# duongve13112002/DiffusionSpatialControl

Measured on AMD Instinct MI355X. Metric: 512x512 images/sec, SD1.5 25-step DPM++2M Karras with region-biased cross-attention, higher is better.
Workload: dtype f16; 1 GPU; SD1.5 512x512, 25-step DPM++2M Karras, CFG 7.5, 2 region masks, 1 image(s) per generation, 2 generation(s) in flight per GPU; images_per_gpu=1, parallelism=dp1 (independent images, no per-step collective), hip_graph=True, outputs_finite=True, full=False

## Files before the change

### diffusionspatialcontrol_amd/_lib.py

```python
import ctypes
import os
import re

_HERE = os.path.dirname(os.path.abspath(__file__))
_LIB = None


class DscLibraryError(RuntimeError):
    pass


def lib_path():
    return os.environ.get("DSC_LIB_PATH") or os.path.join(_HERE, "libdsc_hip.so")


def header_path():
    return os.path.join(os.path.dirname(_HERE), "include", "dsc_hip.h")


def declared_symbols():
    txt = open(header_path()).read()
    txt = re.sub(r"/\*.*?\*/", "", txt, flags=re.S)
    return sorted(set(re.findall(r"\b(dsc_[a-z0-9_]+)\s*\(", txt)))

# ... 47 lines not shown
                                    [ctypes.c_float, ctypes.c_int, ctypes.c_int, _vp, ctypes.c_size_t, _vp]),
    "dsc_set_workspace_slot": (ctypes.c_int, [ctypes.c_int]),
    "dsc_set_tuning_profile": (ctypes.c_int, [ctypes.c_int]),
    "dsc_get_tuning_profile": (ctypes.c_int, []),
    "dsc_linear_lt_stats": (None, [_vp]),
    "dsc_has_library_gemm": (ctypes.c_int, []),
    "dsc_add_bias_residual": (ctypes.c_int, [_vp] * 4 + [ctypes.c_int64, ctypes.c_int, ctypes.c_int, _vp]),
    "dsc_linear_f16": (ctypes.c_int, [_vp] * 5 + [ctypes.c_int64, ctypes.c_int, ctypes.c_int] + [ctypes.c_int64] * 3 +
                       [ctypes.c_int, ctypes.c_int, _vp]),
    "dsc_debug_set_conv_stamps": (None, [_vp]),
    "dsc_debug_set_conv_ring": (None, [ctypes.c_int]),
    "dsc_conv3x3_supported": (ctypes.c_int, [ctypes.c_int] * 5),
    "dsc_conv3x3_workspace_bytes": (ctypes.c_size_t, [ctypes.c_int] * 6),
    "dsc_conv3x3_nhwc_f16": (ctypes.c_int, [_vp] * 5 + [ctypes.c_int] * 5 + [ctypes.c_int64] * 3 +
                             [ctypes.c_int, ctypes.c_int, ctypes.c_int, ctypes.c_int, _vp, ctypes.c_size_t, _vp]),
    "dsc_conv3x3_fewcin_f16": (ctypes.c_int, [_vp] * 4 + [ctypes.c_int] * 6 + [_vp]),
    "dsc_linear_lt_f16": (ctypes.c_int, [_vp] * 5 + [ctypes.c_int64, ctypes.c_int, ctypes.c_int] + [ctypes.c_int64] * 3 +
                          [ctypes.c_int, _vp]),
    "dsc_linear_rows_f16": (ctypes.c_int, [_vp] * 4 + [ctypes.c_int] * 3 + [ctypes.c_int64] * 2 + [ctypes.c_int, ctypes.c_int, _vp]),
    "dsc_linear_ln_f16": (ctypes.c_int, [_vp] * 5 + [ctypes.c_int64, ctypes.c_int, ctypes.c_int] + [ctypes.c_int64] * 3 +
                          [ctypes.c_int, _vp, ctypes.c_int, _vp, ctypes.c_float, _vp, ctypes.c_int, _vp]),
    "dsc_debug_set_gemm_stages": (None, [ctypes.c_int]),
    "dsc_linear_qkv_f16": (ctypes.c_int, [_vp] * 5 + [ctypes.c_int64, ctypes.c_int, ctypes.c_int, ctypes.c_int64, ctypes.c_int64,
                                          ctypes.c_int, ctypes.c_int, _vp, ctypes.c_int, _vp, ctypes.c_float, ctypes.c_int, _vp]),
    "dsc_add_layernorm": (ctypes.c_int, [_vp] * 6 + [ctypes.c_int64, ctypes.c_int, ctypes.c_float, ctypes.c_int, _vp]),
    "dsc_geglu": (ctypes.c_int, [_vp, _vp, ctypes.c_int64, ctypes.c_int, ctypes.c_int, _vp]),
    "dsc_linear_splitk_workspace_bytes": (ctypes.c_size_t, [ctypes.c_int64, ctypes.c_int, ctypes.c_int, ctypes.c_int]),
    "dsc_linear_splitk_f16": (ctypes.c_int, [_vp] * 5 + [ctypes.c_int64, ctypes.c_int, ctypes.c_int] + [ctypes.c_int64] * 3 +
                              [ctypes.c_int, _vp, ctypes.c_size_t, ctypes.c_int, _vp]),
    "dsc_conv3x3_gn_rows": (ctypes.c_int, [ctypes.c_int] * 7),
# ... 56 lines not shown
```

### diffusionspatialcontrol_amd/csrc/conv3x3.hip

```cpp
#include "dsc_common.h"
#include "dsc_hip.h"
#include "gn_partials.h"
#include <type_traits>

extern int g_dsc_tuning_profile;

namespace {

constexpr int BM = 128, BN = 64, BK = 64, T = 256;
constexpr int kBStageBytes = BN * BK * 2;
constexpr int kAPiecesMax = 25;
constexpr int kABytes = kAPiecesMax * 1024;
constexpr int kRingOff = 0;
constexpr int a_off(int S) { return S * kBStageBytes; }
constexpr int pad_off(int S) { return a_off(S) + 2 * kABytes; }
constexpr int lds_bytes(int S) { return pad_off(S) + 1024; }
constexpr int kEpiStride = BN + 4;
constexpr unsigned kOob = 0x80000000u;

struct ConvParams {
    const half_t* x; const half_t* w; const half_t* bias; const half_t* res; half_t* out; float* ws;
    int B, H, W, Cin, Cout;
    int up;
    int sh, sw;
    int nchw;
    int sub2;
    int oh, ow;
    long long onpix;
    long long ldx, ldr, ldo;
    int nc, splits, cps;
    int order;
// ... 7 lines not shown
    const half_t* add; long long add_ld;
    float* gn_part; int gn_cpg, gn_G;
};

__device__ __forceinline__ void dma16(__amdgpu_buffer_rsrc_t rsrc, unsigned voff, unsigned soff, unsigned lds_byte) {
    __builtin_amdgcn_raw_ptr_buffer_load_lds(rsrc, (__attribute__((address_space(3))) void*)(uintptr_t)lds_byte, 16, voff, soff, 0, 0);
}

template <int N>
__device__ __forceinline__ void wait_vm() {
    static_assert(N >= 0 && N < 64, "vmcnt is 6 bits");
    __builtin_amdgcn_s_waitcnt((N & 15) | (7 << 4) | (15 << 8) | ((N >> 4) << 14));
    asm volatile("" ::: "memory");
}

template <int S>
constexpr int younger_dmas(int t) {
    int n = 0;
    for (int i = 1; i <= S - 2; ++i) n += ((t - i) % 9 + 9) % 9 == 0 ? 9 : 2;
    return n;
}
template <int S>
__device__ __forceinline__ void wait_step(int t) {
    switch (t) {
        case 0: wait_vm<younger_dmas<S>(0)>(); break;
        case 1: wait_vm<younger_dmas<S>(1)>(); break;
        case 2: wait_vm<younger_dmas<S>(2)>(); break;
        case 3: wait_vm<younger_dmas<S>(3)>(); break;
        case 4: wait_vm<younger_dmas<S>(4)>(); break;
        case 5: wait_vm<younger_dmas<S>(5)>(); break;
        case 6: wait_vm<younger_dmas<S>(6)>(); break;
        case 7: wait_vm<younger_dmas<S>(7)>(); break;
        default: wait_vm<younger_dmas<S>(8)>(); break;
    }
}

template <int TW>
__device__ __forceinline__ int halo_swz(int hy, int hx) {
    if constexpr (TW == 16) return (hx >> 1) & 7;
    else return ((hx >> 1) ^ ((hy & 1) << 2)) & 7;
}

struct Frags { h8_t w[4], x0[4], x1[4]; };

__device__ __forceinline__ h8_t lds_read(unsigned byte_addr) {
    return *reinterpret_cast<const __attribute__((address_space(3))) h8_t*>((uintptr_t)byte_addr);
}

template <int TW, int S, int NLOAD = 0>
__global__ __launch_bounds__(T + 64 * NLOAD, (S == 3 || NLOAD ? 2 : 1)) void conv3x3_kernel(ConvParams p) {
    static_assert(S == 3 || S == 9, "the ring depth must divide the 9 taps");
    static_assert(NLOAD == 0 || NLOAD == 4, "loader waves mirror the four computing waves' DMA shares");
    constexpr bool LOADER = NLOAD > 0;
    constexpr int kAOff = a_off(S), kPadOff = pad_off(S);
    constexpr int NSB = 16 / TW;
    constexpr int HWD = TW + 2;
    constexpr int HS = 10 * HWD;
    constexpr int NSLOT = NSB * HS;
    constexpr int NPIECE = (NSLOT + 7) / 8;
    constexpr int NPAR = TW == 16 ? 1 : 2;
    constexpr int MT1 = (32 / TW) * HWD * 128;
    static_assert(NPIECE <= kAPiecesMax && NPIECE <= 28, "halo does not fit");

    extern __shared__ __attribute__((aligned(16))) char smem[];

    const int lane = threadIdx.x & 63, wave_all = __builtin_amdgcn_readfirstlane(threadIdx.x >> 6);
    const bool is_loader = LOADER && wave_all >= 4;
    const int wave = wave_all & 3;
    const int r = lane & 31, hh = lane >> 5;
    const int wm = wave >> 1, wn = wave & 1;

    const int total = p.mt * p.nt * p.splits;
    const int per = gridDim.x >> 3;
    const int v = (blockIdx.x & 7) * per + (blockIdx.x >> 3);
    if (v >= total) return;
    long long st0 = 0, st1 = 0, st2 = 0, sc0 = 0, sc1 = 0, sc2 = 0;
    if (p.stamps) { st0 = __builtin_amdgcn_s_memrealtime(); sc0 = __builtin_amdgcn_s_memtime(); }
    int bm, bn, sp;
    if (p.order) {
        const int rest = fdiv(v, p.fd_nt);
        bn = v - rest * p.nt;
        sp = fdiv(rest, p.fd_mt); bm = rest - sp * p.mt;
    } else {
        const int rest = fdiv(v, p.fd_mt);
        bm = v - rest * p.mt;
        sp = fdiv(rest, p.fd_nt); bn = rest - sp * p.nt;
    }
    const int n0 = bn * BN;
    const int cb = sp * p.cps, ce = min(p.nc, cb + p.cps);
    const int ns = (ce - cb) * 9;

    const __amdgpu_buffer_rsrc_t xr = __builtin_amdgcn_make_buffer_rsrc(const_cast<half_t*>(p.x), 0, p.x_bytes, 0x00020000);
    const __amdgpu_buffer_rsrc_t wr = __builtin_amdgcn_make_buffer_rsrc(const_cast<half_t*>(p.w), 0, p.w_bytes, 0x00020000);

    unsigned wvoff[2];
#pragma unroll
    for (int pc = 0; pc < 2; ++pc) {
        const int row = (pc * 4 + wave) * 8 + (lane >> 3);
        const int chunk = (lane & 7) ^ ((row >> 1) & 7);
        wvoff[pc] = ((unsigned)(n0 + row) * 9u * (unsigned)p.Cin + chunk * 8) * 2u;
    }
    auto issue_b = [&](unsigned soff, int stage) {
#pragma unroll
        for (int pc = 0; pc < 2; ++pc) dma16(wr, wvoff[pc], soff, kRingOff + stage * kBStageBytes + (pc * 4 + wave) * 1024);
    };
    auto tile_soff = [&](int c, int t) { return ((unsigned)t * (unsigned)p.Cin + (unsigned)c * BK) * 2u; };

    const bool dma_wave = !LOADER || is_loader;
    if (dma_wave) {
#pragma unroll
        for (int k = 0; k < S; ++k) issue_b(tile_soff(cb, k), k);
    }

    int ob[NSB], oy[NSB], ox[NSB];
#pragma unroll
// ... 11 lines not shown
        if (slot < NSLOT) {
            const int sb = slot / HS, rem = slot % HS;
            const int hy = rem / HWD, hx = rem % HWD;
            const int b = NSB == 1 ? ob[0] : (sb ? ob[NSB - 1] : ob[0]);
            const int y = (NSB == 1 ? oy[0] : (sb ? oy[NSB - 1] : oy[0])) - 1 + hy;
            const int x = (NSB == 1 ? ox[0] : (sb ? ox[NSB - 1] : ox[0])) - 1 + hx;
            if (b >= 0 && y >= 0 && y < p.H && x >= 0 && x < p.W) {
                const int px = p.up ? (b * p.sh + (y >> 1)) * p.sw + (x >> 1) : (b * p.H + y) * p.W + x;
                off = ((unsigned)px * (unsigned)p.ldx + (((lane & 7) ^ halo_swz<TW>(hy, hx)) << 3)) * 2u;
            }
        }
        aoff[i] = off;
    }
    auto issue_a = [&](int i, int c, int ab) {
        const int piece = i * 4 + wave;
        const unsigned dst = piece < NPIECE ? kAOff + ab * kABytes + piece * 1024 : kPadOff;
        dma16(xr, aoff[i], (unsigned)c * (BK * 2), dst);
    };
    unsigned xaddr[NPAR][3][4], waddr[4], waddr_hi[4];
    {
        const int m = wm * 64 + r;
        const int sb = m / (8 * TW), py = (m % (8 * TW)) / TW, pxl = m % TW;
        const int slot00 = sb * HS + py * HWD + pxl;
#pragma unroll
        for (int par = 0; par < NPAR; ++par)
#pragma unroll
            for (int dx = 0; dx < 3; ++dx) {
                const int sw = halo_swz<TW>(py + par, pxl + dx);
#pragma unroll
                for (int ks = 0; ks < 4; ++ks) xaddr[par][dx][ks] = (unsigned)(kAOff + (slot00 + dx) * 128 + (((2 * ks + hh) ^ sw) << 4));
            }
        const int wrow = wn * 32 + r;
#pragma unroll
        for (int ks = 0; ks < 4; ++ks) {
            waddr[ks] = (unsigned)(kRingOff + wrow * 128 + (((2 * ks + hh) ^ ((wrow >> 1) & 7)) << 4));
            waddr_hi[ks] = waddr[ks] + 4 * kBStageBytes;
        }
    }
    auto load_frags = [&](Frags& f, int ab, int t) {
        const int dy = t / 3, dx = t % 3;
        const unsigned abase = ab * kABytes + dy * HWD * 128;
        const int stg = t % S;
#pragma unroll
        for (int ks = 0; ks < 4; ++ks) {
            f.w[ks] = stg < 4 ? lds_read(waddr[ks] + stg * kBStageBytes) : lds_read(waddr_hi[ks] + (stg - 4) * kBStageBytes);
            f.x0[ks] = lds_read(xaddr[NPAR == 1 ? 0 : (dy & 1)][dx][ks] + abase);
            f.x1[ks] = lds_read(xaddr[NPAR == 1 ? 0 : (dy & 1)][dx][ks] + abase + MT1);
        }
    };

    f16x_t acc[2];
#pragma unroll
    for (int i = 0; i < 16; ++i) { acc[0][i] = 0.f; acc[1][i] = 0.f; }

    if (dma_wave) {
#pragma unroll
        for (int i = 0; i < 7; ++i) issue_a(i, cb, 0);
    }
    wait_vm<0>();
    __builtin_amdgcn_s_barrier();
    if constexpr (LOADER) {
        if (is_loader) {
            for (int c = cb; c < ce; ++c) {
                const int jb = (c - cb) * 9;
                const int cn = c + 1 < ce ? c + 1 : c;
                const int P = (c - cb) & 1;
#pragma unroll
                for (int t = 0; t < 9; ++t) {
                    wait_step<S>(t);
                    __builtin_amdgcn_s_barrier();
                    if (t == 0) {
#pragma unroll
                        for (int i = 0; i < 7; ++i) issue_a(i, cn, P ^ 1);
                    }
                    const bool more = jb + t + S < ns;
                    const int c3 = t + S >= 9 ? c + 1 : c, t3 = (t + S) % 9;
                    issue_b(more ? tile_soff(c3, t3) : tile_soff(c, t), t % S);
                }
            }
            __syncthreads();
            __syncthreads();
            if (p.gn_part) dsc_gn::gn_tile_partials_barriers();
            return;
        }
    }
    Frags f[2];
    load_frags(f[0], 0, 0);
    if (p.stamps) { st1 = __builtin_amdgcn_s_memrealtime(); sc1 = __builtin_amdgcn_s_memtime(); }

    auto slice = [&](auto parity, int c) {
        constexpr int P = decltype(parity)::value;
        const int jb = (c - cb) * 9;
        const int cn = c + 1 < ce ? c + 1 : c;
#pragma unroll
        for (int t = 0; t < 9; ++t) {
            Frags& cur = f[(P + t) & 1];
            Frags& nxt = f[(P + t + 1) & 1];
            if (!LOADER) wait_step<S>(t);
            asm volatile("s_waitcnt lgkmcnt(0)" ::: "memory");
            __builtin_amdgcn_s_barrier();
            __builtin_amdgcn_sched_barrier(0);
            if (!LOADER) {
                if (t == 0) {
#pragma unroll
                    for (int i = 0; i < 7; ++i) issue_a(i, cn, P ^ 1);
                }
                const bool more = jb + t + S < ns;
                const int c3 = t + S >= 9 ? c + 1 : c, t3 = (t + S) % 9;
                issue_b(more ? tile_soff(c3, t3) : tile_soff(c, t), t % S);
            }
            if (t < 8) load_frags(nxt, P, t + 1);
            else load_frags(nxt, P ^ 1, 0);
#pragma unroll
            for (int ks = 0; ks < 4; ++ks) {
                acc[0] = mfma_32x32x16(cur.w[ks], cur.x0[ks], acc[0]);
                acc[1] = mfma_32x32x16(cur.w[ks], cur.x1[ks], acc[1]);
            }
            if (!LOADER) __builtin_amdgcn_sched_group_barrier(0x20, 1, 0);
#pragma unroll
            for (int g = 0; g < 8; ++g) {
                if (g < 6) __builtin_amdgcn_sched_group_barrier(0x100, 2, 0);
                __builtin_amdgcn_sched_group_barrier(0x8, 1, 0);
                if (!LOADER && g < (t == 0 ? 8 : 1)) __builtin_amdgcn_sched_group_barrier(0x20, 1, 0);
            }
            __builtin_amdgcn_sched_barrier(0);
        }
// ... 32 lines not shown
#pragma unroll
        for (int g = 0; g < 4; ++g) {
            const f4x_t vv = {acc[mt][4 * g], acc[mt][4 * g + 1], acc[mt][4 * g + 2], acc[mt][4 * g + 3]};
            *reinterpret_cast<f4x_t*>(stage + (wm * 64 + mt * 32 + r) * kEpiStride + wn * 32 + 8 * g + 4 * hh) = vv;
        }
    __syncthreads();
#pragma unroll
    for (int cidx = 0; cidx < 4; ++cidx) {
        const int idx = threadIdx.x + cidx * T, m = idx >> 3, ch = idx & 7;
        const int sb = m / (8 * TW), py = (m % (8 * TW)) / TW, pxl = m % TW;
        const int b = NSB == 1 ? ob[0] : (sb ? ob[NSB - 1] : ob[0]);
        if (b < 0) continue;
        const int yy = (NSB == 1 ? oy[0] : (sb ? oy[NSB - 1] : oy[0])) + py, xx = (NSB == 1 ? ox[0] : (sb ? ox[NSB - 1] : ox[0])) + pxl;
        if (yy >= p.H || xx >= p.W) continue;
        long long gp = ((long long)b * p.H + yy) * p.W + xx;
        if (p.sub2) {
            if (p.sub2 == 1 ? ((yy | xx) & 1) != 0 : (yy & xx & 1) == 0) continue;
            gp = ((long long)b * p.oh + (yy >> 1)) * p.ow + (xx >> 1);
        }
        const float* sp_ = stage + m * kEpiStride + ch * 8;
        if (p.splits > 1) {
            float* dst = p.ws + ((long long)sp * p.onpix + gp) * p.Cout + n0 + ch * 8;
            *reinterpret_cast<f4x_t*>(dst) = *reinterpret_cast<const f4x_t*>(sp_);
            *reinterpret_cast<f4x_t*>(dst + 4) = *reinterpret_cast<const f4x_t*>(sp_ + 4);
        } else {
            const int c0 = n0 + ch * 8;
            if (c0 >= p.Cout) continue;
            if (c0 + 8 <= p.Cout && !p.nchw) {
                const h8_t bv = bpre, rv = rpre[cidx];
                h8_t o;
// ... 23 lines not shown
    if (p.gn_part) {
        float* dst = ob[0] >= 0 ? p.gn_part + ((long long)ob[0] * p.bpi + (bm - ob[0] * p.bpi)) * p.gn_G * 4 : nullptr;
        dsc_gn::gn_tile_partials(gs, gq, reinterpret_cast<float*>(smem) + BM * kEpiStride, n0, p.gn_cpg, p.gn_G, dst);
    }
    if (p.stamps && threadIdx.x == 0) {
        unsigned hwid;
        asm volatile("s_getreg_b32 %0, hwreg(HW_REG_HW_ID)" : "=s"(hwid));
        unsigned xcc;
        asm volatile("s_getreg_b32 %0, hwreg(HW_REG_XCC_ID)" : "=s"(xcc));
        long long* o = p.stamps + (long long)v * 8;
        o[0] = st0; o[1] = st1; o[2] = st2; o[3] = __builtin_amdgcn_s_memrealtime();
        o[4] = sc1 - sc0; o[5] = sc2 - sc1; o[6] = __builtin_amdgcn_s_memtime() - sc2; o[7] = ((long long)xcc << 32) | hwid;
    }
}

__global__ __launch_bounds__(256) void conv3x3_reduce(ConvParams p) {
    const int cv = p.Cout >> 3;
    const int idx = blockIdx.x * 256 + threadIdx.x;
    if (idx >= (int)p.onpix * cv) return;
    const int gpi = fdiv(idx, p.fd_cv);
    const long long gp = gpi;
    const int n = (idx - gpi * cv) * 8;
    float s[8] = {0, 0, 0, 0, 0, 0, 0, 0};
    for (int k = 0; k < p.splits; ++k) {
        const float* src = p.ws + ((long long)k * p.onpix + gp) * p.Cout + n;
        const f4x_t a = *reinterpret_cast<const f4x_t*>(src), b = *reinterpret_cast<const f4x_t*>(src + 4);
#pragma unroll
        for (int j = 0; j < 4; ++j) { s[j] += a[j]; s[4 + j] += b[j]; }
    }
    h8_t bv = {0, 0, 0, 0, 0, 0, 0, 0}, rv = {0, 0, 0, 0, 0, 0, 0, 0};
// ... 8 lines not shown
long long* g_conv_stamps = nullptr;
int g_conv_ring = 0;

bool al16(const void* q) { return (reinterpret_cast<uintptr_t>(q) & 15) == 0; }

int tile_width(int H, int W) {
    if (H < 1 || W < 1) return 0;
    if (W % 16 == 0) return 16;
    if (W % 8 == 0) return 8;
    return ((W + 15) / 16 * 16 - W <= (W + 7) / 8 * 8 - W) ? 16 : 8;
}

int g_conv_loaders = 1;
int g_conv_order = -1;
double g_conv_small_step = 0.14;
int auto_splits(int tiles, int nc, long long npix, int cout) {
    int best = 1;
    double best_t = 1e30;
    for (int s = 1; s <= nc; ++s) {
        if (nc % s != 0) continue;
        const long long wgs = (long long)tiles * s;
        if (s > 1 && wgs > 1024) break;
        const double load = wgs <= 256 ? g_conv_small_step / 0.26 : (wgs <= 512 ? 1.15 : 1.15 * (double)wgs / 512.0);
        double t = 9.0 * nc / s * 0.26 * load + 5.0;
        if (s > 1) t += 4.0 + (double)s * (double)npix * cout * 8.0 / 3.0e6;
        if (t < best_t) { best_t = t; best = s; }
    }
    return best;
}

int plan(int B, int H, int W, int Cin, int Cout, int splits, ConvParams* p) {
    const int tw = tile_width(H, W);
    if (!tw || Cin % BK != 0 || Cout <= 0) return 0;
    p->B = B; p->H = H; p->W = W; p->Cin = Cin; p->Cout = Cout;
    p->nc = Cin / BK;
    p->bpr = (W + tw - 1) / tw; p->bpi = ((H + 7) / 8) * p->bpr; p->nblk = B * p->bpi;
    const int nsb = 16 / tw;
    p->mt = (p->nblk + nsb - 1) / nsb; p->nt = (Cout + BN - 1) / BN;
    p->npix = (long long)B * H * W;
    if (Cout % BN != 0) splits = 1;
    if (splits <= 0) splits = auto_splits(p->mt * p->nt, p->nc, p->npix, Cout);
    if (splits > p->nc) splits = p->nc;
    p->cps = (p->nc + splits - 1) / splits;
    p->splits = (p->nc + p->cps - 1) / p->cps;
    const long long total = (long long)p->mt * p->nt * p->splits;
    p->fd_mt = make_fastdiv(p->mt, total); p->fd_nt = make_fastdiv(p->nt, total);
    p->fd_bpi = make_fastdiv(p->bpi, (long long)p->mt * nsb + nsb); p->fd_bpr = make_fastdiv(p->bpr, p->bpi);
    return tw;
}

}

extern "C" void dsc_debug_set_conv_stamps(void* device_buffer) { g_conv_stamps = static_cast<long long*>(device_buffer); }

extern "C" void dsc_debug_set_conv_ring(int stages) {
    if (stages >= 400) g_conv_loaders = stages - 400;
    else if (stages >= 300) g_conv_order = stages - 300;
    else if (stages >= 200) g_conv_small_step = (stages - 200) / 100.0;
    else g_conv_ring = stages;
}

extern "C" int dsc_conv3x3_supported(int B, int H, int W, int Cin, int Cout) {
    ConvParams p{};
    if (B <= 0 || H <= 0 || W <= 0 || (long long)B * H * W * (long long)(Cin > Cout ? Cin : Cout) >= (1ll << 30) ||
        9ll * Cin * Cout >= (1ll << 30)) return 0;
    return plan(B, H, W, Cin, Cout, 0, &p) ? 1 : 0;
}

extern "C" size_t dsc_conv3x3_workspace_bytes(int B, int H, int W, int Cin, int Cout, int splits) {
    ConvParams p{};
    if (B <= 0 || H <= 0 || W <= 0 || !plan(B, H, W, Cin, Cout, splits, &p)) return 0;
// ... 100 lines not shown
    } else {
        if (loaders) DSC_LAUNCH((conv3x3_kernel<8, 9, 4>), grid, block8, (size_t)lds_bytes(9), st, p);
        else if (ring == 9) DSC_LAUNCH((conv3x3_kernel<8, 9>), grid, block, (size_t)lds_bytes(9), st, p);
        else DSC_LAUNCH((conv3x3_kernel<8, 3>), grid, block, (size_t)lds_bytes(3), st, p);
    }
    if (hipGetLastError() != hipSuccess) return DSC_ERR_LAUNCH;
    if (p.splits > 1) {
        const long long n = p.onpix * (Cout / 8);
        p.fd_cv = make_fastdiv(Cout / 8, n + 256);
        DSC_LAUNCH(conv3x3_reduce, dim3((unsigned)((n + 255) / 256)), dim3(256), 0, st, p);
        if (hipGetLastError() != hipSuccess) return DSC_ERR_LAUNCH;
    }
    return DSC_OK;
}
}
```

### diffusionspatialcontrol_amd/modules/u_net_condition_modify.py

```python
import inspect
import math
from dataclasses import dataclass, field
from typing import Any, Dict, Optional, Tuple

import torch
import torch.nn as nn
import torch.nn.functional as F

from .. import ops
from .attention_modify import AttnProcessor, AttnProcessor2_0


class ImageProjection(nn.Module):

    def __init__(self, image_embed_dim=768, cross_attention_dim=768, num_image_text_embeds=32):
        super().__init__()
        self.num_image_text_embeds = num_image_text_embeds
        self.image_embeds = nn.Linear(image_embed_dim, num_image_text_embeds * cross_attention_dim)
        self.norm = nn.LayerNorm(cross_attention_dim)

    def forward(self, image_embeds):
        b = image_embeds.shape[0]
        return self.norm(self.image_embeds(image_embeds).reshape(b, self.num_image_text_embeds, -1))

# ... 490 lines not shown
        super().__init__()
        self.conv = nn.Conv2d(c, c, 3, stride=2, padding=1)

    def forward(self, x):
        if ops.conv3x3_supported(x, self.conv.weight):
            return ops.conv3x3(x, self.conv.weight, self.conv.bias, stride2_ceil=True)
        return self.conv(x)


class Upsample2D(nn.Module):
    def __init__(self, c):
        super().__init__()
        self.conv = nn.Conv2d(c, c, 3, padding=1)

    def forward(self, x, output_size=None):
        if output_size is None:
            if ops.conv3x3_supported(x, self.conv.weight, upsample=True):
                return ops.conv3x3(x, self.conv.weight, self.conv.bias, upsample=True)
            return self.conv(F.interpolate(x, scale_factor=2.0, mode="nearest"))
        output_size = tuple(int(v) for v in output_size)
        if all(t in (2 * s_, 2 * s_ - 1) for t, s_ in zip(output_size, x.shape[2:])) \
                and ops.conv3x3_supported(x, self.conv.weight, upsample_size=output_size):
            return ops.conv3x3(x, self.conv.weight, self.conv.bias, upsample_size=output_size)
        return self.conv(F.interpolate(x, size=output_size, mode="nearest"))


class _Block(nn.Module):

    def __init__(self, res_io, temb_dim, cfg, heads, depth, down=False, up=False):
        super().__init__()
        cout = res_io[-1][1]
        self.resnets = nn.ModuleList([ResnetBlock2D(i, o, temb_dim, cfg.norm_num_groups, cfg.norm_eps) for i, o in res_io])
        self.has_attn = depth > 0
        if self.has_attn:
            self.attentions = nn.ModuleList([
# ... 270 lines not shown
```

### diffusionspatialcontrol_amd/ops.py

```python
import ctypes
import os

import numpy as np
import torch

from . import _lib

FLAG_REF_FP16_ROUNDING = 1
FLAG_BIAS_IS_FINAL = 2
FLAG_REUSE_STATS = 4
FLAG_ROWS_PADDED = 256
FLAG_SIGMA_PER_GROUP = 512
REGION_ROW_STRIDE = 100

def _stream_ptr(t):
    return ctypes.c_void_p(torch.cuda.current_stream(t.device).cuda_stream)


def _p(t):
    return ctypes.c_void_p(t.data_ptr()) if t is not None else None


def _i64x3(a, b, c):
    return (ctypes.c_int64 * 3)(a, b, c)
# ... 715 lines not shown
    if residual is not None:
        if residual.shape != out.shape:
            raise ValueError("conv3x3: residual must have the output's shape")
        if not residual.is_contiguous(memory_format=cl):
            residual = residual.contiguous(memory_format=cl)
        ldr = Cout
    nbytes = lib.dsc_conv3x3_workspace_bytes(B, H, W, Cin, Cout, splits)
    ws = _workspace(x.device, nbytes) if nbytes else None
    rc = lib.dsc_conv3x3_nhwc_f16(_p(x), _p(weight), _p(bias), _p(residual), _p(out), B, H, W, Cin, Cout, Cin, ldr, Cout,
                                  3 if stride2_pad_br else (2 if stride2 else (1 if upsample else (4 if size is not None else 0))), 1 if out_nchw else 0, splits, 0, _p(ws),
                                  ws.numel() * 8 if ws is not None else 0, _stream_ptr(x))
    _lib.check(rc, "dsc_conv3x3_nhwc_f16")
    return out


def conv3x3_fewcin(x, weight_t, bias, cout):
    _require_gpu(x, weight_t)
    x = x.contiguous()
    B, Cin, H, W = x.shape
    out = torch.empty((B, cout, H, W), dtype=x.dtype, device=x.device, memory_format=torch.channels_last)
    rc = _lib.load_library().dsc_conv3x3_fewcin_f16(_p(x), _p(weight_t), _p(bias), _p(out), B, Cin, H, W, cout, 0, _stream_ptr(x))
    _lib.check(rc, "dsc_conv3x3_fewcin_f16")
    return out


def linear_rows(x, weight, bias=None, silu_out=False, sinusoid_dim=0):
    _require_gpu(x, weight)
    N, K = weight.shape
    if sinusoid_dim:
        if x.dtype != torch.float32 or x.dim() != 1 or sinusoid_dim != K:
# ... 286 lines not shown
```

### include/dsc_hip.h

```cpp
#ifndef DSC_HIP_H
#define DSC_HIP_H

#include <stddef.h>
#include <stdint.h>

#ifdef __cplusplus
extern "C" {
#endif

#define DSC_OK                0
#define DSC_ERR_BAD_ARG      -1
#define DSC_ERR_UNSUPPORTED  -2
#define DSC_ERR_WORKSPACE    -3
#define DSC_ERR_LAUNCH       -4

#define DSC_F16 0
#define DSC_FLAG_REF_FP16_ROUNDING 1u
#define DSC_FLAG_REUSE_STATS       4u
#define DSC_FLAG_ROWS_PADDED     256u
#define DSC_FLAG_BIAS_IS_FINAL     2u
#define DSC_FLAG_SIGMA_PER_GROUP 512u

int dsc_abi_version(void);
const char* dsc_target_arch(void);
// ... 115 lines not shown
                   int64_t M, int N, int K, int64_t ldx, int64_t ldr, int64_t ldo, int geglu, int dtype, void* stream);

#define DSC_CONV_UPSAMPLE2X 1
#define DSC_CONV_STRIDE2 2
#define DSC_CONV_STRIDE2_PAD_BR 3
#define DSC_CONV_UPSAMPLE_CEIL 4
int dsc_conv3x3_supported(int B, int H, int W, int Cin, int Cout);
void dsc_debug_set_conv_stamps(void* device_buffer);
void dsc_debug_set_conv_ring(int stages);
size_t dsc_conv3x3_workspace_bytes(int B, int H, int W, int Cin, int Cout, int splits);
int dsc_conv3x3_nhwc_f16(const void* x, const void* w, const void* bias, const void* residual, void* out,
                         int B, int H, int W, int Cin, int Cout, int64_t ldx, int64_t ldr, int64_t ldo,
                         int resample, int out_nchw, int splits, int dtype, void* workspace, size_t workspace_bytes,
                         void* stream);

int dsc_linear_ln_f16(const void* x, const void* w, const void* bias, const void* residual, void* out,
                      int64_t M, int N, int K, int64_t ldx, int64_t ldr, int64_t ldo, int geglu,
                      const float* ln_in, int ln_nb, const float* ln_cvec, float ln_eps, float* ln_out,
                      int dtype, void* stream);
void dsc_debug_set_gemm_stages(int stages);
int dsc_linear_qkv_f16(const void* x, const void* w, const void* bias, void* q_out, void* kv_out,
                       int64_t M, int C, int K, int64_t ldx, int64_t ldq, int heads, int seq_len,
                       const float* ln_in, int ln_nb, const float* ln_cvec, float ln_eps, int dtype, void* stream);

int dsc_conv3x3_fewcin_f16(const void* x_nchw, const void* w_t, const void* bias, void* out_nhwc,
                           int B, int Cin, int H, int W, int Cout, int dtype, void* stream);

int dsc_linear_lt_f16(const void* x, const void* w, const void* bias, const void* residual, void* out,
                      int64_t M, int N, int K, int64_t ldx, int64_t ldr, int64_t ldo, int dtype, void* stream);
int dsc_has_library_gemm(void);
// ... 46 lines not shown
```

Measured before the change: 11.63 images/s.

## Decompose nearest-2x upsample conv into four 2x2 phase convolutions

Adds a phase-decomposed form of the nearest-upsample-then-3x3-conv used in SD1.5 upsample blocks. Weights are pre-summed into four 2x2 kernels, one per output phase, and the conv kernel body is templated on tap count so each phase tile runs 4 taps on the low-resolution input instead of 9 taps on the upsampled image. This cuts MAC work and input traffic for the upsample convs by more than half. In exchange it adds a cached packed-weight tensor, fp16 rounding of the summed weights, and a new split heuristic for the up2x path.

Result: faster. 11.79 images/s, median of 6 (+1.3%).

```diff
diff --git a/diffusionspatialcontrol_amd/_lib.py b/diffusionspatialcontrol_amd/_lib.py
--- a/diffusionspatialcontrol_amd/_lib.py
+++ b/diffusionspatialcontrol_amd/_lib.py
@@ -85,6 +85,11 @@
     "dsc_conv3x3_workspace_bytes": (ctypes.c_size_t, [ctypes.c_int] * 6),
     "dsc_conv3x3_nhwc_f16": (ctypes.c_int, [_vp] * 5 + [ctypes.c_int] * 5 + [ctypes.c_int64] * 3 +
                              [ctypes.c_int, ctypes.c_int, ctypes.c_int, ctypes.c_int, _vp, ctypes.c_size_t, _vp]),
+    "dsc_conv3x3_up2x_pack_f16": (ctypes.c_int, [_vp, _vp, ctypes.c_int, ctypes.c_int, _vp]),
+    "dsc_conv3x3_up2x_supported": (ctypes.c_int, [ctypes.c_int] * 5),
+    "dsc_conv3x3_up2x_workspace_bytes": (ctypes.c_size_t, [ctypes.c_int] * 6),
+    "dsc_conv3x3_up2x_nhwc_f16": (ctypes.c_int, [_vp] * 4 + [ctypes.c_int] * 6 + [_vp, ctypes.c_size_t, ctypes.c_int64, ctypes.c_int64,
+                                                                                   ctypes.c_int, _vp]),
     "dsc_conv3x3_fewcin_f16": (ctypes.c_int, [_vp] * 4 + [ctypes.c_int] * 6 + [_vp]),
     "dsc_linear_lt_f16": (ctypes.c_int, [_vp] * 5 + [ctypes.c_int64, ctypes.c_int, ctypes.c_int] + [ctypes.c_int64] * 3 +
                           [ctypes.c_int, _vp]),
diff --git a/diffusionspatialcontrol_amd/csrc/conv3x3.hip b/diffusionspatialcontrol_amd/csrc/conv3x3.hip
--- a/diffusionspatialcontrol_amd/csrc/conv3x3.hip
+++ b/diffusionspatialcontrol_amd/csrc/conv3x3.hip
@@ -15,6 +15,8 @@
 constexpr int a_off(int S) { return S * kBStageBytes; }
 constexpr int pad_off(int S) { return a_off(S) + 2 * kABytes; }
 constexpr int lds_bytes(int S) { return pad_off(S) + 1024; }
+constexpr int a_bytes(int NT, int TW) { return NT == 4 && TW == 16 ? 23 * 1024 : kABytes; }
+constexpr int lds_bytes_up2x(int TW) { return a_off(4) + 2 * a_bytes(4, TW) + 1024; }
 constexpr int kEpiStride = BN + 4;
 constexpr unsigned kOob = 0x80000000u;
 
@@ -52,24 +54,24 @@
     asm volatile("" ::: "memory");
 }
 
-template <int S>
+template <int S, int NT>
 constexpr int younger_dmas(int t) {
     int n = 0;
-    for (int i = 1; i <= S - 2; ++i) n += ((t - i) % 9 + 9) % 9 == 0 ? 9 : 2;
+    for (int i = 1; i <= S - 2; ++i) n += ((t - i) % NT + NT) % NT == 0 ? 9 : 2;
     return n;
 }
-template <int S>
+template <int S, int NT>
 __device__ __forceinline__ void wait_step(int t) {
     switch (t) {
-        case 0: wait_vm<younger_dmas<S>(0)>(); break;
-        case 1: wait_vm<younger_dmas<S>(1)>(); break;
-        case 2: wait_vm<younger_dmas<S>(2)>(); break;
-        case 3: wait_vm<younger_dmas<S>(3)>(); break;
-        case 4: wait_vm<younger_dmas<S>(4)>(); break;
-        case 5: wait_vm<younger_dmas<S>(5)>(); break;
-        case 6: wait_vm<younger_dmas<S>(6)>(); break;
-        case 7: wait_vm<younger_dmas<S>(7)>(); break;
-        default: wait_vm<younger_dmas<S>(8)>(); break;
+        case 0: wait_vm<younger_dmas<S, NT>(0)>(); break;
+        case 1: wait_vm<younger_dmas<S, NT>(1)>(); break;
+        case 2: wait_vm<younger_dmas<S, NT>(2)>(); break;
+        case 3: wait_vm<younger_dmas<S, NT>(3)>(); break;
+        case 4: wait_vm<younger_dmas<S, NT>(4)>(); break;
+        case 5: wait_vm<younger_dmas<S, NT>(5)>(); break;
+        case 6: wait_vm<younger_dmas<S, NT>(6)>(); break;
+        case 7: wait_vm<younger_dmas<S, NT>(7)>(); break;
+        default: wait_vm<younger_dmas<S, NT>(8)>(); break;
     }
 }
 
@@ -85,12 +87,16 @@
     return *reinterpret_cast<const __attribute__((address_space(3))) h8_t*>((uintptr_t)byte_addr);
 }
 
-template <int TW, int S, int NLOAD = 0>
-__global__ __launch_bounds__(T + 64 * NLOAD, (S == 3 || NLOAD ? 2 : 1)) void conv3x3_kernel(ConvParams p) {
-    static_assert(S == 3 || S == 9, "the ring depth must divide the 9 taps");
+template <int TW, int S, int NLOAD, int NT>
+__device__ __forceinline__ void conv3x3_body(const ConvParams& p) {
+    static_assert(NT == 9 || NT == 4, "nine taps, or the four of a phase of the 2x-upsampled form");
+    static_assert(NT % S == 0, "the ring depth must divide the taps of a slice (a tile's stage is its tap % S)");
     static_assert(NLOAD == 0 || NLOAD == 4, "loader waves mirror the four computing waves' DMA shares");
+    static_assert(NT == 9 || NLOAD == 0, "the phase form has no loader-wave variant");
     constexpr bool LOADER = NLOAD > 0;
-    constexpr int kAOff = a_off(S), kPadOff = pad_off(S);
+    constexpr bool UP = NT == 4;
+    constexpr int kAB = a_bytes(NT, TW);
+    constexpr int kAOff = a_off(S), kPadOff = kAOff + 2 * kAB;
     constexpr int NSB = 16 / TW;
     constexpr int HWD = TW + 2;
     constexpr int HS = 10 * HWD;
@@ -98,7 +104,7 @@
     constexpr int NPIECE = (NSLOT + 7) / 8;
     constexpr int NPAR = TW == 16 ? 1 : 2;
     constexpr int MT1 = (32 / TW) * HWD * 128;
-    static_assert(NPIECE <= kAPiecesMax && NPIECE <= 28, "halo does not fit");
+    static_assert(NPIECE * 1024 <= kAB && NPIECE <= 28, "halo does not fit");
 
     extern __shared__ __attribute__((aligned(16))) char smem[];
 
@@ -126,7 +132,14 @@
     }
     const int n0 = bn * BN;
     const int cb = sp * p.cps, ce = min(p.nc, cb + p.cps);
-    const int ns = (ce - cb) * 9;
+    const int ns = (ce - cb) * NT;
+    int phase = 0;
+    if constexpr (UP) {
+        const int mts = p.mt >> 2;
+        phase = (bm >= mts) + (bm >= 2 * mts) + (bm >= 3 * mts);
+        bm -= phase * mts;
+    }
+    const int PY = phase >> 1, PX = phase & 1;
 
     const __amdgpu_buffer_rsrc_t xr = __builtin_amdgcn_make_buffer_rsrc(const_cast<half_t*>(p.x), 0, p.x_bytes, 0x00020000);
     const __amdgpu_buffer_rsrc_t wr = __builtin_amdgcn_make_buffer_rsrc(const_cast<half_t*>(p.w), 0, p.w_bytes, 0x00020000);
@@ -136,7 +149,7 @@
     for (int pc = 0; pc < 2; ++pc) {
         const int row = (pc * 4 + wave) * 8 + (lane >> 3);
         const int chunk = (lane & 7) ^ ((row >> 1) & 7);
-        wvoff[pc] = ((unsigned)(n0 + row) * 9u * (unsigned)p.Cin + chunk * 8) * 2u;
+        wvoff[pc] = ((unsigned)(phase * p.Cout + n0 + row) * (unsigned)NT * (unsigned)p.Cin + chunk * 8) * 2u;
     }
     auto issue_b = [&](unsigned soff, int stage) {
 #pragma unroll
@@ -178,18 +191,19 @@
     }
     auto issue_a = [&](int i, int c, int ab) {
         const int piece = i * 4 + wave;
-        const unsigned dst = piece < NPIECE ? kAOff + ab * kABytes + piece * 1024 : kPadOff;
+        const unsigned dst = piece < NPIECE ? kAOff + ab * kAB + piece * 1024 : kPadOff;
         dma16(xr, aoff[i], (unsigned)c * (BK * 2), dst);
     };
-    unsigned xaddr[NPAR][3][4], waddr[4], waddr_hi[4];
+    constexpr int NDX = UP ? 2 : 3;
+    unsigned xaddr[NPAR][NDX][4], waddr[4], waddr_hi[4];
     {
         const int m = wm * 64 + r;
-        const int sb = m / (8 * TW), py = (m % (8 * TW)) / TW, pxl = m % TW;
+        const int sb = m / (8 * TW), py = (m % (8 * TW)) / TW + PY, pxl = m % TW + PX;
         const int slot00 = sb * HS + py * HWD + pxl;
 #pragma unroll
         for (int par = 0; par < NPAR; ++par)
 #pragma unroll
-            for (int dx = 0; dx < 3; ++dx) {
+            for (int dx = 0; dx < NDX; ++dx) {
                 const int sw = halo_swz<TW>(py + par, pxl + dx);
 #pragma unroll
                 for (int ks = 0; ks < 4; ++ks) xaddr[par][dx][ks] = (unsigned)(kAOff + (slot00 + dx) * 128 + (((2 * ks + hh) ^ sw) << 4));
@@ -202,8 +216,8 @@
         }
     }
     auto load_frags = [&](Frags& f, int ab, int t) {
-        const int dy = t / 3, dx = t % 3;
-        const unsigned abase = ab * kABytes + dy * HWD * 128;
+        const int dy = t / NDX, dx = t % NDX;
+        const unsigned abase = ab * kAB + dy * HWD * 128;
         const int stg = t % S;
 #pragma unroll
         for (int ks = 0; ks < 4; ++ks) {
@@ -226,19 +240,19 @@
     if constexpr (LOADER) {
         if (is_loader) {
             for (int c = cb; c < ce; ++c) {
-                const int jb = (c - cb) * 9;
+                const int jb = (c - cb) * NT;
                 const int cn = c + 1 < ce ? c + 1 : c;
                 const int P = (c - cb) & 1;
 #pragma unroll
-                for (int t = 0; t < 9; ++t) {
-                    wait_step<S>(t);
+                for (int t = 0; t < NT; ++t) {
+                    wait_step<S, NT>(t);
                     __builtin_amdgcn_s_barrier();
                     if (t == 0) {
 #pragma unroll
                         for (int i = 0; i < 7; ++i) issue_a(i, cn, P ^ 1);
                     }
                     const bool more = jb + t + S < ns;
-                    const int c3 = t + S >= 9 ? c + 1 : c, t3 = (t + S) % 9;
+                    const int c3 = t + S >= NT ? c + 1 : c, t3 = (t + S) % NT;
                     issue_b(more ? tile_soff(c3, t3) : tile_soff(c, t), t % S);
                 }
             }
@@ -254,13 +268,14 @@
 
     auto slice = [&](auto parity, int c) {
         constexpr int P = decltype(parity)::value;
-        const int jb = (c - cb) * 9;
+        constexpr int FP = (NT & 1) ? P : 0;
+        const int jb = (c - cb) * NT;
         const int cn = c + 1 < ce ? c + 1 : c;
 #pragma unroll
-        for (int t = 0; t < 9; ++t) {
-            Frags& cur = f[(P + t) & 1];
-            Frags& nxt = f[(P + t + 1) & 1];
-            if (!LOADER) wait_step<S>(t);
+        for (int t = 0; t < NT; ++t) {
+            Frags& cur = f[(FP + t) & 1];
+            Frags& nxt = f[(FP + t + 1) & 1];
+            if (!LOADER) wait_step<S, NT>(t);
             asm volatile("s_waitcnt lgkmcnt(0)" ::: "memory");
             __builtin_amdgcn_s_barrier();
             __builtin_amdgcn_sched_barrier(0);
@@ -270,10 +285,10 @@
                     for (int i = 0; i < 7; ++i) issue_a(i, cn, P ^ 1);
                 }
                 const bool more = jb + t + S < ns;
-                const int c3 = t + S >= 9 ? c + 1 : c, t3 = (t + S) % 9;
+                const int c3 = t + S >= NT ? c + 1 : c, t3 = (t + S) % NT;
                 issue_b(more ? tile_soff(c3, t3) : tile_soff(c, t), t % S);
             }
-            if (t < 8) load_frags(nxt, P, t + 1);
+            if (t < NT - 1) load_frags(nxt, P, t + 1);
             else load_frags(nxt, P ^ 1, 0);
 #pragma unroll
             for (int ks = 0; ks < 4; ++ks) {
@@ -336,6 +351,7 @@
         const int yy = (NSB == 1 ? oy[0] : (sb ? oy[NSB - 1] : oy[0])) + py, xx = (NSB == 1 ? ox[0] : (sb ? ox[NSB - 1] : ox[0])) + pxl;
         if (yy >= p.H || xx >= p.W) continue;
         long long gp = ((long long)b * p.H + yy) * p.W + xx;
+        if constexpr (UP) gp = ((long long)b * (2 * p.H) + (2 * yy + PY)) * (2 * p.W) + (2 * xx + PX);
         if (p.sub2) {
             if (p.sub2 == 1 ? ((yy | xx) & 1) != 0 : (yy & xx & 1) == 0) continue;
             gp = ((long long)b * p.oh + (yy >> 1)) * p.ow + (xx >> 1);
@@ -389,6 +405,16 @@
     }
 }
 
+template <int TW, int S, int NLOAD = 0>
+__global__ __launch_bounds__(T + 64 * NLOAD, (S == 3 || NLOAD ? 2 : 1)) void conv3x3_kernel(ConvParams p) {
+    conv3x3_body<TW, S, NLOAD, 9>(p);
+}
+
+template <int TW>
+__global__ __launch_bounds__(T, (TW == 16 ? 2 : 1)) void conv3x3_kernel_up2x(ConvParams p) {
+    conv3x3_body<TW, 4, 0, 4>(p);
+}
+
 __global__ __launch_bounds__(256) void conv3x3_reduce(ConvParams p) {
     const int cv = p.Cout >> 3;
     const int idx = blockIdx.x * 256 + threadIdx.x;
@@ -427,22 +453,25 @@
 int g_conv_loaders = 1;
 int g_conv_order = -1;
 double g_conv_small_step = 0.14;
-int auto_splits(int tiles, int nc, long long npix, int cout) {
+double g_up2x_small_step = 0.14;
+int auto_splits(int tiles, int nc, long long npix, int cout, int taps, int per_cu) {
     int best = 1;
     double best_t = 1e30;
     for (int s = 1; s <= nc; ++s) {
         if (nc % s != 0) continue;
         const long long wgs = (long long)tiles * s;
         if (s > 1 && wgs > 1024) break;
-        const double load = wgs <= 256 ? g_conv_small_step / 0.26 : (wgs <= 512 ? 1.15 : 1.15 * (double)wgs / 512.0);
-        double t = 9.0 * nc / s * 0.26 * load + 5.0;
+        const double small = (taps == 4 ? g_up2x_small_step : g_conv_small_step) / 0.26;
+        const double load = wgs <= 256 ? small : (per_cu == 1 ? small * (double)((wgs + 255) / 256)
+                                                              : (wgs <= 512 ? 1.15 : 1.15 * (double)wgs / 512.0));
+        double t = (double)taps * nc / s * 0.26 * load + 5.0;
         if (s > 1) t += 4.0 + (double)s * (double)npix * cout * 8.0 / 3.0e6;
         if (t < best_t) { best_t = t; best = s; }
     }
     return best;
 }
 
-int plan(int B, int H, int W, int Cin, int Cout, int splits, ConvParams* p) {
+int plan(int B, int H, int W, int Cin, int Cout, int splits, ConvParams* p, int taps = 9) {
     const int tw = tile_width(H, W);
     if (!tw || Cin % BK != 0 || Cout <= 0) return 0;
     p->B = B; p->H = H; p->W = W; p->Cin = Cin; p->Cout = Cout;
@@ -451,8 +480,10 @@
     const int nsb = 16 / tw;
     p->mt = (p->nblk + nsb - 1) / nsb; p->nt = (Cout + BN - 1) / BN;
     p->npix = (long long)B * H * W;
+    p->onpix = p->npix;
+    if (taps == 4) { p->mt *= 4; p->onpix = 4 * p->npix; }
     if (Cout % BN != 0) splits = 1;
-    if (splits <= 0) splits = auto_splits(p->mt * p->nt, p->nc, p->npix, Cout);
+    if (splits <= 0) splits = auto_splits(p->mt * p->nt, p->nc, p->onpix, Cout, taps, taps == 4 && tw == 8 ? 1 : 2);
     if (splits > p->nc) splits = p->nc;
     p->cps = (p->nc + splits - 1) / splits;
     p->splits = (p->nc + p->cps - 1) / p->cps;
@@ -467,7 +498,8 @@
 extern "C" void dsc_debug_set_conv_stamps(void* device_buffer) { g_conv_stamps = static_cast<long long*>(device_buffer); }
 
 extern "C" void dsc_debug_set_conv_ring(int stages) {
-    if (stages >= 400) g_conv_loaders = stages - 400;
+    if (stages >= 500) g_up2x_small_step = (stages - 500) / 100.0;
+    else if (stages >= 400) g_conv_loaders = stages - 400;
     else if (stages >= 300) g_conv_order = stages - 300;
     else if (stages >= 200) g_conv_small_step = (stages - 200) / 100.0;
     else g_conv_ring = stages;
@@ -598,3 +630,103 @@
     return DSC_OK;
 }
 }
+
+
+namespace {
+
+__global__ __launch_bounds__(256) void conv3x3_up2x_pack_kernel(const half_t* __restrict__ w, half_t* __restrict__ packed, int Cin, int Cout) {
+    const int cv = Cin >> 3;
+    const long long idx = (long long)blockIdx.x * 256 + threadIdx.x;
+    if (idx >= 16ll * Cout * cv) return;
+    const int c = (int)(idx % cv) * 8;
+    const int tap = (int)(idx / cv) & 3;
+    const long long pn = idx / cv / 4;
+    const int n = (int)(pn % Cout), phase = (int)(pn / Cout);
+    const int py = phase >> 1, px = phase & 1, a = tap >> 1, b = tap & 1;
+    const int dy0 = py + a == 0 ? 0 : (py + a == 2 ? 2 : 1 - py), dy1 = py + a == 1 ? dy0 + 1 : dy0;
+    const int dx0 = px + b == 0 ? 0 : (px + b == 2 ? 2 : 1 - px), dx1 = px + b == 1 ? dx0 + 1 : dx0;
+    float s[8];
+    bool first = true;
+    for (int dy = dy0; dy <= dy1; ++dy)
+        for (int dx = dx0; dx <= dx1; ++dx) {
+            const h8_t v = *reinterpret_cast<const h8_t*>(w + ((long long)(n * 3 + dy) * 3 + dx) * Cin + c);
+#pragma unroll
+            for (int j = 0; j < 8; ++j) s[j] = first ? (float)v[j] : s[j] + (float)v[j];
+            first = false;
+        }
+    h8_t o;
+#pragma unroll
+    for (int j = 0; j < 8; ++j) o[j] = (half_t)s[j];
+    *reinterpret_cast<h8_t*>(packed + idx * 8) = o;
+}
+
+bool up2x_shape_ok(int B, int h, int w, int Cin, int Cout) {
+    if (B <= 0 || h <= 0 || w <= 0 || Cin <= 0 || Cout <= 0 || Cin % BK != 0 || Cout % BN != 0) return false;
+    return 4ll * B * h * w * (long long)(Cin > Cout ? Cin : Cout) < (1ll << 30) && 16ll * Cin * Cout < (1ll << 30);
+}
+
+}
+
+extern "C" int dsc_conv3x3_up2x_pack_f16(const void* w, void* packed, int Cin, int Cout, void* stream) {
+    if (!w || !packed || Cin <= 0 || Cout <= 0) return DSC_ERR_BAD_ARG;
+    if (Cin % BK != 0 || 16ll * Cin * Cout >= (1ll << 30) || !al16(w) || !al16(packed)) return DSC_ERR_UNSUPPORTED;
+    const long long n = 16ll * Cout * (Cin / 8);
+    DSC_LAUNCH(conv3x3_up2x_pack_kernel, dim3((unsigned)((n + 255) / 256)), dim3(256), 0, static_cast<hipStream_t>(stream),
+               static_cast<const half_t*>(w), static_cast<half_t*>(packed), Cin, Cout);
+    return hipGetLastError() == hipSuccess ? DSC_OK : DSC_ERR_LAUNCH;
+}
+
+extern "C" int dsc_conv3x3_up2x_supported(int B, int h, int w, int Cin, int Cout) {
+    ConvParams p{};
+    return up2x_shape_ok(B, h, w, Cin, Cout) && plan(B, h, w, Cin, Cout, 0, &p, 4) ? 1 : 0;
+}
+
+extern "C" size_t dsc_conv3x3_up2x_workspace_bytes(int B, int h, int w, int Cin, int Cout, int splits) {
+    ConvParams p{};
+    if (!up2x_shape_ok(B, h, w, Cin, Cout) || !plan(B, h, w, Cin, Cout, splits, &p, 4)) return 0;
+    return p.splits > 1 ? (size_t)p.splits * p.onpix * Cout * sizeof(float) : 0;
+}
+
+extern "C" int dsc_conv3x3_up2x_nhwc_f16(const void* x, const void* w_packed, const void* bias, void* out, int B, int h, int w,
+                                         int Cin, int Cout, int splits, void* workspace, size_t workspace_bytes, int64_t ldx,
+                                         int64_t ldo, int dtype, void* stream) {
+    if (!x || !w_packed || !out || B <= 0 || h <= 0 || w <= 0 || Cin <= 0 || Cout <= 0) return DSC_ERR_BAD_ARG;
+    if (dtype != DSC_F16) return DSC_ERR_UNSUPPORTED;
+    if (ldx < Cin || ldo < Cout) return DSC_ERR_BAD_ARG;
+    if (ldx % 8 != 0 || ldo % 8 != 0) return DSC_ERR_UNSUPPORTED;
+    if (!al16(x) || !al16(w_packed) || !al16(out) || (bias && !al16(bias))) return DSC_ERR_UNSUPPORTED;
+    if (!up2x_shape_ok(B, h, w, Cin, Cout) || 4ll * B * h * w * (ldx > ldo ? ldx : ldo) >= (1ll << 30)) return DSC_ERR_UNSUPPORTED;
+    ConvParams p{};
+    const int tw = plan(B, h, w, Cin, Cout, splits, &p, 4);
+    if (!tw) return DSC_ERR_UNSUPPORTED;
+    p.x = static_cast<const half_t*>(x); p.w = static_cast<const half_t*>(w_packed);
+    p.bias = static_cast<const half_t*>(bias); p.out = static_cast<half_t*>(out); p.ws = static_cast<float*>(workspace);
+    p.ldx = ldx; p.ldo = ldo;
+    p.stamps = g_conv_stamps;
+    p.order = g_conv_order >= 0 ? g_conv_order : (p.onpix >= 2ll * Cout ? 1 : 0);
+    p.x_bytes = (unsigned)(((p.npix - 1) * ldx + Cin) * 2);
+    p.w_bytes = (unsigned)(16ll * Cin * Cout * 2);
+    if (p.splits > 1) {
+        const size_t need = (size_t)p.splits * p.onpix * Cout * sizeof(float);
+        if (!workspace || workspace_bytes < need || !al16(workspace)) return DSC_ERR_WORKSPACE;
+    }
+    hipStream_t st = static_cast<hipStream_t>(stream);
+    static bool attr_set = false;
+    if (!attr_set) {
+        (void)hipFuncSetAttribute(reinterpret_cast<const void*>(&conv3x3_kernel_up2x<16>), hipFuncAttributeMaxDynamicSharedMemorySize, 160 * 1024);
+        (void)hipFuncSetAttribute(reinterpret_cast<const void*>(&conv3x3_kernel_up2x<8>), hipFuncAttributeMaxDynamicSharedMemorySize, 160 * 1024);
+        attr_set = true;
+    }
+    const int total = p.mt * p.nt * p.splits;
+    const dim3 grid(((total + 7) / 8) * 8), block(T);
+    if (tw == 16) DSC_LAUNCH((conv3x3_kernel_up2x<16>), grid, block, (size_t)lds_bytes_up2x(16), st, p);
+    else DSC_LAUNCH((conv3x3_kernel_up2x<8>), grid, block, (size_t)lds_bytes_up2x(8), st, p);
+    if (hipGetLastError() != hipSuccess) return DSC_ERR_LAUNCH;
+    if (p.splits > 1) {
+        const long long n = p.onpix * (Cout / 8);
+        p.fd_cv = make_fastdiv(Cout / 8, n + 256);
+        DSC_LAUNCH(conv3x3_reduce, dim3((unsigned)((n + 255) / 256)), dim3(256), 0, st, p);
+        if (hipGetLastError() != hipSuccess) return DSC_ERR_LAUNCH;
+    }
+    return DSC_OK;
+}
diff --git a/diffusionspatialcontrol_amd/modules/u_net_condition_modify.py b/diffusionspatialcontrol_amd/modules/u_net_condition_modify.py
--- a/diffusionspatialcontrol_amd/modules/u_net_condition_modify.py
+++ b/diffusionspatialcontrol_amd/modules/u_net_condition_modify.py
@@ -528,11 +528,16 @@
         self.conv = nn.Conv2d(c, c, 3, padding=1)
 
     def forward(self, x, output_size=None):
+        if output_size is not None:
+            output_size = tuple(int(v) for v in output_size)
+        if output_size is None or output_size == (2 * x.shape[2], 2 * x.shape[3]):
+            w = self.conv.weight
+            if ops.USE_UP2X_PHASES and ops.conv3x3_up2x_supported(x, w):
+                return ops.conv3x3_up2x(x, _derived(self, "up2x", (w,), lambda: ops.conv3x3_up2x_pack(w)), self.conv.bias)
         if output_size is None:
             if ops.conv3x3_supported(x, self.conv.weight, upsample=True):
                 return ops.conv3x3(x, self.conv.weight, self.conv.bias, upsample=True)
             return self.conv(F.interpolate(x, scale_factor=2.0, mode="nearest"))
-        output_size = tuple(int(v) for v in output_size)
         if all(t in (2 * s_, 2 * s_ - 1) for t, s_ in zip(output_size, x.shape[2:])) \
                 and ops.conv3x3_supported(x, self.conv.weight, upsample_size=output_size):
             return ops.conv3x3(x, self.conv.weight, self.conv.bias, upsample_size=output_size)
diff --git a/diffusionspatialcontrol_amd/ops.py b/diffusionspatialcontrol_amd/ops.py
--- a/diffusionspatialcontrol_amd/ops.py
+++ b/diffusionspatialcontrol_amd/ops.py
@@ -753,6 +753,58 @@
     return out
 
 
+USE_UP2X_PHASES = os.environ.get("DSC_UP2X_PHASES", "1") != "0"
+
+
+def conv3x3_up2x_pack(weight):
+    _require_gpu(weight)
+    if weight.dim() != 4 or tuple(weight.shape[2:]) != (3, 3) or weight.dtype != torch.float16:
+        raise ValueError("conv3x3_up2x_pack: weight must be a [Cout, Cin, 3, 3] fp16 tensor")
+    Cout, Cin = weight.shape[:2]
+    if Cin % 64 != 0:
+        raise ValueError("conv3x3_up2x_pack: Cin must be a multiple of 64")
+    cl = torch.channels_last
+    if not weight.is_contiguous(memory_format=cl):
+        weight = weight.contiguous(memory_format=cl)
+    packed = torch.empty((4, Cout, 4, Cin), dtype=torch.float16, device=weight.device)
+    rc = _lib.load_library().dsc_conv3x3_up2x_pack_f16(_p(weight), _p(packed), Cin, Cout, _stream_ptr(weight))
+    _lib.check(rc, "dsc_conv3x3_up2x_pack_f16")
+    return packed
+
+
+def conv3x3_up2x_supported(x, weight):
+    if not (USE_DSC_CONV and x.is_cuda and x.dtype == torch.float16 and weight.dtype == torch.float16 and x.dim() == 4
+            and weight.dim() == 4 and tuple(weight.shape[2:]) == (3, 3) and weight.shape[1] == x.shape[1]):
+        return False
+    B, C, h, w = x.shape
+    return bool(_lib.load_library().dsc_conv3x3_up2x_supported(B, h, w, C, weight.shape[0]))
+
+
+def conv3x3_up2x(x, packed, bias=None, splits=0):
+    if x.dim() != 4 or x.dtype != torch.float16:
+        raise ValueError("conv3x3_up2x: x must be a [B, Cin, h, w] fp16 tensor")
+    B, Cin, h, w = x.shape
+    if (packed.dim() != 4 or packed.shape[0] != 4 or packed.shape[2] != 4 or packed.shape[3] != Cin
+            or packed.dtype != torch.float16 or not packed.is_contiguous()):
+        raise ValueError(f"conv3x3_up2x: packed must be the contiguous fp16 [4, Cout, 4, {Cin}] tensor of conv3x3_up2x_pack, "
+                         f"not {tuple(packed.shape)}")
+    Cout = packed.shape[1]
+    if bias is not None and (bias.dtype != torch.float16 or bias.numel() != Cout or not bias.is_contiguous()):
+        raise ValueError("conv3x3_up2x: bias must be a contiguous fp16 [Cout] tensor")
+    _require_gpu(x, packed)
+    lib = _lib.load_library()
+    cl = torch.channels_last
+    if not x.is_contiguous(memory_format=cl):
+        x = x.contiguous(memory_format=cl)
+    out = torch.empty((B, Cout, 2 * h, 2 * w), dtype=x.dtype, device=x.device, memory_format=cl)
+    nbytes = lib.dsc_conv3x3_up2x_workspace_bytes(B, h, w, Cin, Cout, splits)
+    ws = _workspace(x.device, nbytes) if nbytes else None
+    rc = lib.dsc_conv3x3_up2x_nhwc_f16(_p(x), _p(packed), _p(bias), _p(out), B, h, w, Cin, Cout, splits, _p(ws),
+                                       ws.numel() * 8 if ws is not None else 0, Cin, Cout, 0, _stream_ptr(x))
+    _lib.check(rc, "dsc_conv3x3_up2x_nhwc_f16")
+    return out
+
+
 def conv3x3_fewcin(x, weight_t, bias, cout):
     _require_gpu(x, weight_t)
     x = x.contiguous()
diff --git a/include/dsc_hip.h b/include/dsc_hip.h
--- a/include/dsc_hip.h
+++ b/include/dsc_hip.h
@@ -153,6 +153,13 @@
                          int resample, int out_nchw, int splits, int dtype, void* workspace, size_t workspace_bytes,
                          void* stream);
 
+int dsc_conv3x3_up2x_pack_f16(const void* w, void* packed, int Cin, int Cout, void* stream);
+int dsc_conv3x3_up2x_supported(int B, int h, int w, int Cin, int Cout);
+size_t dsc_conv3x3_up2x_workspace_bytes(int B, int h, int w, int Cin, int Cout, int splits);
+int dsc_conv3x3_up2x_nhwc_f16(const void* x, const void* w_packed, const void* bias, void* out, int B, int h, int w,
+                              int Cin, int Cout, int splits, void* workspace, size_t workspace_bytes, int64_t ldx,
+                              int64_t ldo, int dtype, void* stream);
+
 int dsc_linear_ln_f16(const void* x, const void* w, const void* bias, const void* residual, void* out,
                       int64_t M, int N, int K, int64_t ldx, int64_t ldr, int64_t ldo, int geglu,
                       const float* ln_in, int ln_nb, const float* ln_cvec, float ln_eps, float* ln_out,
```
